# mosesyhc/LCGP

Hardware: AMD Instinct MI355X
Metric: NLL+grad evals/sec (higher is better)
Workload: dtype f64; 1 GPU; configs[2]: n=4096 d=6 p=64 q=8 submethod=full, one NLL+gradient evaluation per step; n=4096, d=6, p=64, q=8, parallelism=latent components k -> rank k mod 1, q_local_rank0=8

## Files before the change

### include/lcgp_hip.h

```cpp
#ifndef LCGP_HIP_H
#define LCGP_HIP_H

#include <stddef.h>
#include <stdint.h>

#ifdef __cplusplus
extern "C" {
#endif

#define LCGP_F64 0
#define LCGP_F32 1

#define LCGP_KERNEL_MATERN32 0
#define LCGP_KERNEL_SE 1
#define LCGP_KERNEL_MATERN52 2

int lcgp_version(void);
const char* lcgp_source_hash(void);
const char* lcgp_last_error(void);

int lcgp_theta_width(int d, int p);
int lcgp_out_width(int d, int p);
int lcgp_partial_width(int d, int p, int q_total);

typedef struct lcgp_sched {
    int outer_blocks;
    int syrk_small_tiles;
    int trtri_small_tiles;
    int lauum_small_tiles;
    int trtri_level_small;
    int fill_leaf;
    int fill_step;
    int leaf_in_wide;
    int progressive_tiles;
    int progressive_far;
    int progressive_lauum;
    int pair_tiles;
} lcgp_sched;
int lcgp_sched_default(lcgp_sched* sched );

int lcgp_workspace_bytes(int dtype, int n, int d, int p, int q_local, size_t* bytes );
int lcgp_predict_scratch_bytes(int dtype, int n, int q_local, int n0, size_t* bytes );

int lcgp_matern32(void* stream, int dtype, int n1, int n2, int d,
                  const void* x1, const void* x2,
                  const double* ell , double scale, double nug, int same, void* out);
int lcgp_covmat(void* stream, int dtype, int kernel_id, int n1, int n2, int d,
                const void* x1, const void* x2,
                const double* ell , double scale, double nug, int same, void* out);

int lcgp_kernel_build(void* stream, int dtype, int kernel_id, int n, int d, int p, int q_local,
                      const void* x , const void* sr ,
                      const double* theta, void* workspace);

int lcgp_potrf_logdet(void* stream, int dtype, int n, int d, int p, int q_local, void* workspace,
                      double* half_logdet, int* info, const lcgp_sched* sched ,
                      const void* plan );

int lcgp_potri(void* stream, int dtype, int n, int d, int p, int q_local, void* workspace,
               const lcgp_sched* sched);
// ... 288 lines not shown
```

### lcgp_amd/_hip.py

```python
from __future__ import annotations

import ctypes as C
import os
import subprocess

_HERE = os.path.dirname(os.path.abspath(__file__))
_ROOT = os.path.dirname(_HERE)
LIB_PATH = os.environ.get("LCGP_HIP_LIB") or os.path.join(_HERE, "liblcgp_hip.so")
SRC_PATH = os.path.join(_HERE, "csrc", "lcgp_hip.hip")
HDR_PATH = os.path.join(_ROOT, "include", "lcgp_hip.h")
SCHED_PATH = os.path.join(_HERE, "csrc", "fill_sched.h")
SUBSET_PATH = os.path.join(_HERE, "csrc", "sobol_subset.h")

F64, F32 = 0, 1
KERNELS = {"matern32": 0, "se": 1, "matern52": 2}


class Sched(C.Structure):
    _fields_ = [("outer_blocks", C.c_int), ("syrk_small_tiles", C.c_int), ("trtri_small_tiles", C.c_int),
                ("lauum_small_tiles", C.c_int), ("trtri_level_small", C.c_int), ("fill_leaf", C.c_int),
                ("fill_step", C.c_int), ("leaf_in_wide", C.c_int), ("progressive_tiles", C.c_int), ("progressive_far", C.c_int), ("progressive_lauum", C.c_int), ("pair_tiles", C.c_int)]


_vp, _i, _d = C.c_void_p, C.c_int, C.c_double
_sp = C.POINTER(Sched)
SIGNATURES = {
    "lcgp_version": (_i, []),
    "lcgp_source_hash": (C.c_char_p, []),
    "lcgp_last_error": (C.c_char_p, []),
    "lcgp_theta_width": (_i, [_i, _i]),
    "lcgp_out_width": (_i, [_i, _i]),
    "lcgp_partial_width": (_i, [_i, _i, _i]),
    "lcgp_sched_default": (_i, [_sp]),
    "lcgp_workspace_bytes": (_i, [_i, _i, _i, _i, _i, C.POINTER(C.c_size_t)]),
    "lcgp_predict_scratch_bytes": (_i, [_i, _i, _i, _i, C.POINTER(C.c_size_t)]),
    "lcgp_matern32": (_i, [_vp, _i, _i, _i, _i, _vp, _vp, C.POINTER(_d), _d, _d, _i, _vp]),
    "lcgp_covmat": (_i, [_vp, _i, _i, _i, _i, _i, _vp, _vp, C.POINTER(_d), _d, _d, _i, _vp]),
    "lcgp_kernel_build": (_i, [_vp, _i, _i, _i, _i, _i, _i, _vp, _vp, _vp, _vp]),
    "lcgp_potrf_logdet": (_i, [_vp, _i, _i, _i, _i, _i, _vp, _vp, _vp, _sp, _vp]),
    "lcgp_potri": (_i, [_vp, _i, _i, _i, _i, _i, _vp, _sp]),
    "lcgp_trtri": (_i, [_vp, _i, _i, _i, _i, _i, _vp, _sp]),
    "lcgp_lauum": (_i, [_vp, _i, _i, _i, _i, _i, _vp, _sp]),
    "lcgp_lauum_clock": (_i, [_vp, _i, _i, _i, _i, _i, _vp, _vp]),
    "lcgp_fetch_matrix": (_i, [_vp, _i, _i, _i, _i, _i, _vp, _i, _i, _vp]),
# ... 178 lines not shown
```

### lcgp_amd/csrc/fill_sched.h

```cpp
#ifndef LCGP_FILL_SCHED_H
#define LCGP_FILL_SCHED_H

#include <stddef.h>
#include <string.h>
#include <utility>
#include <vector>

namespace lcgp_fill {

enum FillType { FILL_NONE = 0, FILL_SYRK = 1, FILL_BROW = 2, FILL_CUPD = 3, FILL_DUPD = 4, FILL_TRI_T = 5, FILL_TRI_W = 6 };

constexpr int NJ = 6;

struct FillJob {
    int type;
    int nblk;
    int t0;
    int R0, R1, j0, j1;
    int kb0, kb1;
};

struct FillSet {
    void* M; void* W; void* V;
    size_t mat;
// ... 171 lines not shown
                fs.nblk += o.nblk;
            }
            hi = lo;
            jb.next = jb.total;
        }
        return fs.nblk;
    }

    void end_launch() {
        for (QJob& jb : jobs) jb.avail = jb.next;
        ++launch;
    }
};

struct PlanParams {
    int nb;
    int q;
    int ob;
    int syrk_small_tiles, fill_leaf, fill_step, leaf_in_wide;
    bool progressive;
    bool far_rides;
    bool with_dupd = true;
    int pair_tiles = 0;
};

enum LaunchKind {
    L_LEAF = 1,
    L_STEP = 2,
    L_TRAIL = 3,
    L_FILL = 4
};

struct Launch {
    Launch() { memset((void*)this, 0, sizeof(*this)); }
    int kind = 0;
    int J = 0, pe = 0, c = 0;
    int diag_end = 0, has_special = 0, n_trmm = 0, n_upd = 0;
    int c_lo = 0, c_hi = 0, tiles128 = 0, with_leaf = 0;
    FillSet fs;
};

inline long rect_tiles(int nb, int c_lo, int c_hi) { return syrk_tiles(nb / 2, c_lo, c_hi); }
inline int trapezoid_tiles(int nb, int c_lo, int c_hi) { return (c_hi - c_lo) * nb - (c_lo + c_hi - 1) * (c_hi - c_lo) / 2; }

class Planner {
 public:
    explicit Planner(const PlanParams& p) : pp(p) { fq.q = p.q; }
    std::vector<Launch> launches;
    bool inverse_planned = false;

    void run() {
        const int nb = pp.nb, ob = pp.ob, q = pp.q;
        const bool t128 = (ob & 1) == 0;
        inverse_planned = pp.progressive;
        bool leaf_done = false;
        const int cap_with_leaf = pp.fill_leaf + (ob - 1) * pp.fill_step;
        const int cap_no_leaf = (ob - 1) * pp.fill_step;
        for (int J = 0; J < nb; J += ob) {
            const int pe = J + ob < nb ? J + ob : nb;
            const int mid = pe + ob < nb ? pe + ob : nb;
            auto first_filler_column = [&](int cap_blocks) {
// ... 38 lines not shown
            panel(J, pe, leaf_done, next_leaf);
            if (pe >= nb) break;
            if (pe < c_hi) {
                Launch l;
                l.kind = L_TRAIL; l.J = k_lo; l.pe = pe; l.c_lo = pe; l.c_hi = c_hi;
                l.tiles128 = t128 && (long long)q * trapezoid_tiles(nb / 2, pe / 2, c_hi / 2) >= pp.syrk_small_tiles ? 1 : 0;
                l.with_leaf = next_leaf ? 1 : 0;
                l.fs.njobs = 0; l.fs.nblk = 0;
                launches.push_back(l);
                fq.end_launch();
            }
            leaf_done = next_leaf && pe < c_hi;
            queue_far_update(J, pe, cf);
        }
        int guard = 0;
        while (fq.pending()) {
            Launch l;
            l.kind = L_FILL;
            fq.take_final(l.fs, kb_end);
            if (l.fs.nblk <= 0 || ++guard > 4 * nb + 16) { failed = true; return; }
            launches.push_back(l);
            fq.end_launch();
        }
    }
    bool failed = false;

 private:
    int pair_J = -1, pair_cf = 0;
    PlanParams pp;
    FillQueue fq;
    int urgent_row = 0;
    int last_dupd = -1, last_cupd = -1;
    int kb_end = 0;

    void queue_far_update(int J, int pe, int cf) {
        fq.syrk_job = -1;
        if (cf >= pp.nb) return;
        QJob jb;
        jb.j.type = FILL_SYRK;
        jb.j.R0 = 0; jb.j.R1 = pp.nb / 2; jb.j.j0 = cf; jb.j.j1 = pp.nb; jb.j.kb0 = J; jb.j.kb1 = pe;
        jb.total = syrk_tiles(pp.nb / 2, cf, pp.nb);
        jb.ready_launch = fq.launch;
        fq.syrk_job = fq.add(jb);
    }

    void queue_inverse_jobs(int J, int pe, bool last_step) {
        const int nb = pp.nb;
        const int now = fq.launch;
        int prev = -1;
        for (int mb = 1; mb < pp.ob; mb *= 2) {
// ... 100 lines not shown
```

### lcgp_amd/csrc/lcgp_hip.hip

```cpp
#include <hip/hip_runtime.h>
#include <stdint.h>
#include <stdio.h>
#include <string.h>
#include <math.h>
#include <type_traits>
#include <vector>

#include "../../include/lcgp_hip.h"
#include "fill_sched.h"
#include "sobol_subset.h"

#define LCGP_VERSION 610

namespace {

constexpr int TS = 64;
constexpr int KT = 16;
constexpr int DMAX = 32;
constexpr int DWIDE = 126;

typedef double d4 __attribute__((ext_vector_type(4)));
typedef float f4 __attribute__((ext_vector_type(4)));

thread_local char g_err[256] = "";
// ... 471 lines not shown
    double o;
    asm("s_nop 1\n\tv_mov_b64_dpp %0, %1 row_newbcast:%2 row_mask:0xf bank_mask:0xf" : "=v"(o) : "v"(x), "n"(C));
    return o;
}

template <int C>
__device__ __forceinline__ void fmac_row_bcast(double& acc, double u, double v) {
    asm("v_fmac_f64_dpp %0, %1, %2 row_newbcast:%3 row_mask:0xf bank_mask:0xf" : "+v"(acc) : "v"(u), "v"(v), "n"(C));
}

template <int S, int C>
struct PivotCols {
    static __device__ __forceinline__ void run(double (&rD)[16], double (&rL)[16], double vD, double vL) {
        if constexpr (C < 16) {
            fmac_row_bcast<C>(rD[C], rD[S], vD);
            fmac_row_bcast<C>(rL[C], rD[S], vL);
            PivotCols<S, C + 1>::run(rD, rL, vD, vL);
        }
    }
};

template <int S>
struct PivotSteps {
    static __device__ __forceinline__ void run(double (&rD)[16], double (&rL)[16], double& dmine, int i) {
        if constexpr (S < 16) {
            const double dp = row_bcast<S>(rD[S]);
            dmine = i == S ? rD[S] : dmine;
            const double rdp = fast_rcp(dp);
            const double vD = -rD[S] * rdp, vL = -rL[S] * rdp;
            PivotCols<S, S + 1>::run(rD, rL, vD, vL);
            PivotSteps<S + 1>::run(rD, rL, dmine, i);
        }
    }
};

template <int S>
struct ScaleCols {
    static __device__ __forceinline__ void run(double (&rD)[16], double (&rL)[16], double rsl) {
        if constexpr (S < 16) {
            const double f = row_bcast<S>(rsl);
            rD[S] *= f;
            rL[S] *= f;
            ScaleCols<S + 1>::run(rD, rL, rsl);
        }
    }
};

__device__ __forceinline__ double fast_rsqrt(double a) {
    double y = __builtin_amdgcn_rsq(a);
    double e = fma(-(a * y), y, 1.0);
    y = fma(0.5 * y, e, y);
    e = fma(-(a * y), y, 1.0);
    y = fma(0.5 * y, e, y);
    return y;
// ... 75 lines not shown
            acc[rb][e] = rb < wv ? 0.0 : FROM_LDS ? w[rb * 16 + lq + 4 * e][wv * 16 + li]
                                                  : (double)Mb[(size_t)(rb * 16 + lq + 4 * e) * npad + wv * 16 + li];
    double (*S)[17] = (double (*)[17])scratch;
    int first_bad = 0;
#pragma unroll 1
    for (int kb = 0; kb < 4; ++kb) {
        if (wv == kb) {
#pragma unroll
            for (int rb = 0; rb < 4; ++rb)
#pragma unroll
                for (int e = 0; e < 4; ++e)
                    if (rb >= kb) S[rb * 16 + lq + 4 * e][li] = acc[rb][e];
            const int nlow = 3 - kb;
            const int base = kb * 16;
            double rD[16], rL[16];
            const int lrow = lq < nlow ? base + 16 * (1 + lq) + li : base + li;
#pragma unroll
            for (int c = 0; c < 16; ++c) {
                rD[c] = S[base + li][c];
                const double below = S[lrow][c];
                rL[c] = lq < nlow ? below : 0.0;
            }
            double dmine = 1.0;
            PivotSteps<0>::run(rD, rL, dmine, li);
            const double rsl = fast_rsqrt(dmine);
            ScaleCols<0>::run(rD, rL, rsl);
            if (lq == 0) { dinv[base + li] = rsl; pivs[base + li] = dmine; }
            const unsigned long long bm = __ballot(!(dmine > 0.0)) & 0xffffull;
            if (bm) first_bad = jb * TS + base + __ffsll((long long)bm);
            const int row = lq < nlow ? base + 16 * (1 + lq) + li : lq == nlow ? base + li : 16 * (lq - nlow - 1) + li;
#pragma unroll
            for (int m = 0; m < 16; ++m)
                lt[base + m][row] = lq < nlow ? rL[m] : (lq == nlow && li >= m) ? rD[m] : 0.0;
            if (lane == 0) bad[kb] = first_bad;
        } else if (wv == kb - 1) {
            const int a = kb - 1;
            leaf_inverse_diag(lt, w, dinv, a, lane);
            for (int b = 0; b < a; ++b) {
                const d4 tacc = leaf_inverse_t(lt, w, a, b, lane);
                leaf_inverse_w(w, tacc, a, b, lane);
            }
        } else if (kb == 0) {
            if ((jb & 1) == 0)
                for (int i = wv - 1; i < TS; i += 3) Wb[(size_t)i * npad + TS + lane] = (T)0;
        } else if (wv == ((kb + 1) & 3)) {
            leaf_store_l_panel<T>(Mb, npad, lt, kb - 1, lane);
        } else if (kb >= 2 && wv == ((kb + 2) & 3)) {
// ... 52 lines not shown

template <typename T>
__global__ __launch_bounds__(256, 2) void leaf_kernel(T* __restrict__ M, T* __restrict__ W, size_t mat, int npad, int jb,
                                                   double* __restrict__ logdet, int* __restrict__ info) {
    __shared__ __align__(16) unsigned char lds[LEAF_LDS_BYTES];
    leaf_body<T>(lds, blockIdx.x, M, W, mat, npad, jb, logdet, info);
}

enum GemmOp { OP_SYRK = 1, OP_TRTRI_T = 2, OP_TRTRI_W = 3, OP_LAUUM = 4, OP_PRED_U = 5, OP_PRED_COV = 6, OP_PRED_V = 7, OP_VR = 8,
              OP_VG_P = 9, OP_VG_G = 10, OP_HESS_G = 11, OP_COND_CROSS = 12, OP_COND_U = 13 };
enum Lay { MK = 0, KM = 1 };

struct GemmArgs {
    const void* A; const void* B; void* C;
    size_t sA, sB, sC;
    int ldA, ldB, ldC;
    int nb;
    int p0, p1, p2, p3;
    int q;
    int t0;
    int skipq;
    const void* bvec = nullptr;
    double* part = nullptr;
    unsigned long long* clk = nullptr;
    const double* theta = nullptr;
    const void* xa = nullptr;
    const void* xb = nullptr;
    const double* wref = nullptr;
    const double* gvc = nullptr;
    int ldg = 0, d = 0, kern = 0, tw = 0, nrep = 1, ldp = 0;
};

template <typename T>
__device__ __forceinline__ constexpr int lds_swz(int k) { return (k & 12) * (int)(8 / sizeof(T)); }
static_assert(KT == 16, "lds_swz assumes 16 k rows per stage");
template <typename T>
__device__ __forceinline__ int swz_col(int g16, int l15, int kk) {
    return (g16 ^ (lds_swz<T>(4 * kk) & ~15)) + (l15 ^ (lds_swz<T>(4 * kk) & 15));
}

template <typename T, int L, int TM, int NT>
__device__ __forceinline__ void load_stage(const T* __restrict__ P, int ld, int ks, T (&reg)[TM * KT / NT], int tid) {
    constexpr int EPT = TM * KT / NT;
    if (L == MK) {
        constexpr int TPR = KT / EPT;
        const int m = tid / TPR, kk = (tid % TPR) * EPT;
// ... 220 lines not shown
            }
        }
#pragma unroll
    for (int ni = 0; ni < MIN; ++ni) {
        s[ni] += __shfl_xor(s[ni], 16);
        s[ni] += __shfl_xor(s[ni], 32);
    }
    if (wave >= 2 && lane < 16) {
#pragma unroll
        for (int ni = 0; ni < MIN; ++ni) red[wn0 + ni * 16 + l15] = s[ni];
    }
    __syncthreads();
    if (wave < 2 && lane < 16) {
        const double rd = 1.0 / (D * (double)g.nrep);
        double* part = (double*)g.C + ((size_t)k * ((g.p2 + TM - 1) / TM) + rt) * g.ldp;
#pragma unroll
        for (int ni = 0; ni < MIN; ++ni) {
            const int cl = wn0 + ni * 16 + l15, c = c0 + cl;
            if (c < g.p3) part[c] = (s[ni] + red[cl]) / (fmax(g.gvc[(size_t)k * g.ldg + c], 0.0) + rd);
        }
    }
}

template <typename T, int OP, int TM, int NW>
__device__ __forceinline__ void gemm_body(const GemmArgs& g, const int lin ,
                                          unsigned char* lds) {
    constexpr int LA = (OP == OP_LAUUM) ? KM : MK;
    constexpr int LB = (OP == OP_TRTRI_T || OP == OP_TRTRI_W || OP == OP_LAUUM || OP == OP_PRED_V || OP == OP_VG_G || OP == OP_HESS_G ||
                        OP == OP_COND_U) ? KM : MK;
    constexpr int NT = NW * 64;
    constexpr int LD = TM + 16;
    constexpr int WTM = TM / (NW / 2), WTN = TM / 2;
    constexpr int MIM = WTM / 16, MIN = WTN / 16;
    constexpr int EPT = TM * KT / NT;
    T* As = (T*)lds;
    T* Bs = As + 2 * KT * LD;

    int lin_ = lin;
    if constexpr (OP == OP_TRTRI_T || OP == OP_TRTRI_W || OP == OP_LAUUM) {
        if (g.q < 4 && !g.skipq && ((lin >> 8) & 1)) {
            const int base = lin & ~255, nblk = (int)gridDim.x;
            const int top = base + 255 < nblk ? base + 255 : nblk - 1;
            lin_ = top - (lin - base);
        }
    }
    const int k = lin_ % g.q;
    const int bid = lin_ / g.q;
    const T* Ab = (const T*)g.A + (size_t)k * g.sA;
    const T* Bb = (const T*)g.B + (size_t)k * g.sB;
    T* Cb = (T*)g.C + (size_t)k * g.sC;

    const T* A0; const T* B0; T* Ct;
    ptrdiff_t dA, dB;
    int nkt;
    double alpha = 1.0;
    bool accumulate = false;
    bool tri_b = false;
    if constexpr (OP == OP_SYRK) {
        constexpr int SB = 8;
        int t = bid + g.t0, r;
        int i0 = 0;
        for (;;) {
            const int rows = g.nb - g.p2 - i0 < SB ? g.nb - g.p2 - i0 : SB;
            int cnt = 0;
            for (int i = i0; i < i0 + rows; ++i) cnt += (i < g.p3 - g.p2 ? i : g.p3 - g.p2 - 1) + 1;
            if (t < cnt) break;
            t -= cnt;
            i0 += SB;
        }
        const int rows = g.nb - g.p2 - i0 < SB ? g.nb - g.p2 - i0 : SB;
        int j = 0;
        for (;;) {
            const int lo = j > i0 ? j : i0;
            const int cnt = i0 + rows - lo;
            if (t < cnt) { r = g.p2 + lo + t; break; }
            t -= cnt;
            ++j;
        }
        const int c = g.p2 + j;
        A0 = Ab + (size_t)r * TM * g.ldA + (size_t)g.p0 * TM; dA = TM;
        B0 = Bb + (size_t)c * TM * g.ldB + (size_t)g.p0 * TM; dB = TM;
        nkt = g.p1 - g.p0;
        Ct = Cb + (size_t)r * TM * g.ldC + (size_t)c * TM;
        alpha = -1.0; accumulate = true;
    } else if constexpr (OP == OP_TRTRI_T || OP == OP_TRTRI_W) {
        const int mb = g.p0;
        const int npair = g.p1;
        const int pr = g.p2 + bid % npair, rem = bid / npair;
        int rl, cl;
        if constexpr (OP == OP_TRTRI_T) { cl = rem / mb; rl = rem - cl * mb; }
        else { rl = mb - 1 - rem / mb; cl = rem % mb; }
        const int C0 = 2 * pr * mb, R0 = C0 + mb;
        if (R0 + rl >= g.nb) return;
        if constexpr (OP == OP_TRTRI_T) {
            A0 = Ab + (size_t)(R0 + rl) * TM * g.ldA + (size_t)(C0 + mb - 1) * TM; dA = -(ptrdiff_t)TM;
            B0 = Bb + (size_t)(C0 + mb - 1) * TM * g.ldB + (size_t)(C0 + cl) * TM; dB = -(ptrdiff_t)TM * g.ldB;
            nkt = mb - cl;
        } else {
            A0 = Ab + (size_t)(R0 + rl) * TM * g.ldA + (size_t)R0 * TM; dA = TM;
            B0 = Bb + (size_t)R0 * TM * g.ldB + (size_t)(C0 + cl) * TM; dB = (ptrdiff_t)TM * g.ldB;
            nkt = rl + 1;
            alpha = -1.0;
        }
        Ct = Cb + (size_t)(R0 + rl) * TM * g.ldC + (size_t)(C0 + cl) * TM;
    } else if constexpr (OP == OP_LAUUM) {
        int r, c;
// ... 229 lines not shown
    }
    if constexpr (OP == OP_VR) {
        const int ct = bid % g.p1, rt = bid / g.p1;
        if (g.kern == 0) vr_epilogue<T, 0, TM, MIM, MIN>(g, acc, k, rt, ct, tid, wm0, wn0, lds);
        else if (g.kern == 1) vr_epilogue<T, 1, TM, MIM, MIN>(g, acc, k, rt, ct, tid, wm0, wn0, lds);
        else vr_epilogue<T, 2, TM, MIM, MIN>(g, acc, k, rt, ct, tid, wm0, wn0, lds);
        return;
    }
    if constexpr (OP == OP_PRED_COV) alpha = -g.theta[(size_t)k * g.p1 + g.p2];
    if constexpr (OP == OP_COND_CROSS) alpha = -g.theta[(size_t)k * g.p2 + g.p3];
#pragma unroll
    for (int mi = 0; mi < MIM; ++mi)
#pragma unroll
        for (int ni = 0; ni < MIN; ++ni)
#pragma unroll
            for (int e = 0; e < 4; ++e) {
                const unsigned dvoff = cvoff + ni * 16 * (unsigned)sizeof(T), dsoff = c_soff(mi, e);
                if constexpr (OP == OP_SYRK && TM == 128) {
                    if (g.skipq && bid + g.t0 == 0 && wm0 + mi * 16 + Mfma<T>::row(lane, e) < TS && wn0 + ni * 16 + (lane & 15) < TS)
                        continue;
                }
                if constexpr (PRELOAD_C) {
                    BufIo<T>::store((T)acc[mi][ni][e], crs, dvoff, dsoff);
                } else {
                    double v = alpha * (double)acc[mi][ni][e];
                    if (accumulate) v += (double)BufIo<T>::load(crs, dvoff, dsoff);
                    BufIo<T>::store((T)v, crs, dvoff, dsoff);
                }
            }
    if constexpr (OP == OP_LAUUM || OP == OP_SYRK) {
        if (g.clk && lin == 0 && wave == 0) {
            const unsigned long long c1 = __builtin_amdgcn_s_memtime() - clk0, r1 = __builtin_amdgcn_s_memrealtime() - rt0;
            if (lane == 0) { g.clk[0] = c1; g.clk[1] = r1; }
        }
    }
    if constexpr (OP == OP_LAUUM && TM == 128) {
        if (g.part) {
            __syncthreads();
            double* bsh = (double*)lds;
            double* p1s = bsh + 256;
            double* p2s = p1s + 256;
            int r, c;
            tri_decode(bid, r, c);
            const T* bk = (const T*)g.bvec + (size_t)k * g.ldC;
            if (tid < 256) bsh[tid] = (double)bk[(size_t)(tid < 128 ? r : c) * 128 + (tid & 127)];
            __syncthreads();
// ... 189 lines not shown
        const int ks = own ? 2 * R : kb0;
        rect_tile<T, KM, KM, false>(W + (size_t)ks * TS * ld + (size_t)R * 128, ld, W + (size_t)ks * TS * ld + (size_t)j * TS, ld,
                                    V + (size_t)R * 128 * ld + (size_t)j * TS, ld, (kb1 - ks) * (TS / KT), own, lds);
    }
}

constexpr int FILL_LDS_BYTES = 2 * KT * (128 + 16 + 64 + 16) * 8;

template <typename T>
__global__ __launch_bounds__(256, 2) void fill_kernel(FillSet fs) {
    __shared__ __align__(16) unsigned char lds[FILL_LDS_BYTES];
    fill_dispatch<T>(fs, blockIdx.x, lds);
}

template <typename T>
__global__ __launch_bounds__(256, 2) void leaf_fill_kernel(T* __restrict__ M, T* __restrict__ W, size_t mat, int npad, int jb,
                                                        double* __restrict__ logdet, int* __restrict__ info,
                                                        int q, FillSet fs) {
    __shared__ __align__(16) unsigned char lds[LEAF_LDS_BYTES];
    if ((int)blockIdx.x < q) leaf_body<T>(lds, blockIdx.x, M, W, mat, npad, jb, logdet, info);
    else fill_dispatch<T>(fs, blockIdx.x - q, lds);
}

struct StepArgs {
    void* M; void* W; size_t mat; int npad; int nb;
    int c, J, pe;
    int diag_end;
    int q;
    int has_special;
    int n_trmm;
    int n_upd;
    int trmm_r0, upd_r0;
    double* logdet; int* info;
    FillSet fs;
};

template <typename T>
struct Tile64 {
    typedef typename Mfma<T>::acc_t acc_t;
    static constexpr int LD = TS + 16, NT = 256, EPT = TS * KT / NT, SPT = TS / KT;
    static __device__ __forceinline__ void load(acc_t (&acc)[2][2], const T* Ct, int ld, int lane, int wm0, int wn0) {
#pragma unroll
        for (int i = 0; i < 2; ++i)
#pragma unroll
            for (int j = 0; j < 2; ++j)
#pragma unroll
                for (int e = 0; e < 4; ++e)
                    acc[i][j][e] = Ct[(size_t)(wm0 + i * 16 + Mfma<T>::row(lane, e)) * ld + wn0 + j * 16 + (lane & 15)];
    }
    static __device__ __forceinline__ void zero(acc_t (&acc)[2][2]) {
#pragma unroll
        for (int i = 0; i < 2; ++i)
#pragma unroll
            for (int j = 0; j < 2; ++j)
#pragma unroll
                for (int e = 0; e < 4; ++e) acc[i][j][e] = 0;
    }
    static __device__ __forceinline__ void store(const acc_t (&acc)[2][2], T* Ct, int ld, int lane, int wm0, int wn0) {
#pragma unroll
// ... 26 lines not shown
                T af[2], bf[2];
#pragma unroll
                for (int i = 0; i < 2; ++i) {
                    const T v = as[krow + wm0 + swz_col<T>(i * 16, lane & 15, kk)];
                    af[i] = NEG ? -v : v;
                }
#pragma unroll
                for (int j = 0; j < 2; ++j) bf[j] = bs[krow + wn0 + swz_col<T>(j * 16, lane & 15, kk)];
#pragma unroll
                for (int i = 0; i < 2; ++i)
#pragma unroll
                    for (int j = 0; j < 2; ++j) acc[i][j] = Mfma<T>::run(af[i], bf[j], acc[i][j]);
            }
        }
    }
    template <bool NEG>
    static __device__ __forceinline__ void mma(acc_t (&acc)[2][2], const T* A0, int ldA, const T* B0, int ldB, T* lds,
                                               int tid, int lane, int wm0, int wn0) {
        T pa[SPT][EPT], pb[SPT][EPT];
        fetch(pa, A0, ldA, tid);
        fetch(pb, B0, ldB, tid);
        mma_regs<NEG>(acc, pa, pb, lds, tid, lane, wm0, wn0);
    }
    static __device__ __forceinline__ void to_operand(const acc_t (&acc)[2][2], T* F, int lane, int wm0, int wn0) {
#pragma unroll
        for (int i = 0; i < 2; ++i)
#pragma unroll
            for (int j = 0; j < 2; ++j)
#pragma unroll
                for (int e = 0; e < 4; ++e)
                    F[(wn0 + j * 16 + (lane & 15)) * LD + ((wm0 + i * 16 + Mfma<T>::row(lane, e)) ^ (lane & 15))] = acc[i][j][e];
    }
    template <bool NEG>
    static __device__ __forceinline__ void mma_a_lds(acc_t (&acc)[2][2], const T* F, const T (&pb)[SPT][EPT], T* Bs, int tid,
                                                     int lane, int wm0, int wn0) {
#pragma unroll
        for (int s = 0; s < SPT; ++s) {
            store_stage<T, MK, TS, NT>(Bs + (s & 1) * KT * LD, pb[s], tid);
            __syncthreads();
            const T* as = F + s * KT * LD;
            const T* bs = Bs + (s & 1) * KT * LD;
#pragma unroll
            for (int kk = 0; kk < KT / 4; ++kk) {
                const int krow = (kk * 4 + (lane >> 4)) * LD;
                T af[2], bf[2];
#pragma unroll
                for (int i = 0; i < 2; ++i) {
                    const T v = as[krow + wm0 + i * 16 + ((lane & 15) ^ (4 * kk + (lane >> 4)))];
                    af[i] = NEG ? -v : v;
                }
#pragma unroll
                for (int j = 0; j < 2; ++j) bf[j] = bs[krow + wn0 + swz_col<T>(j * 16, lane & 15, kk)];
#pragma unroll
                for (int i = 0; i < 2; ++i)
#pragma unroll
                    for (int j = 0; j < 2; ++j) acc[i][j] = Mfma<T>::run(af[i], bf[j], acc[i][j]);
            }
        }
    }
    template <bool NEG>
    static __device__ __forceinline__ void mma_ab_lds(acc_t (&acc)[2][2], const T* F, int lane, int wm0, int wn0) {
#pragma unroll
        for (int kk = 0; kk < TS / 4; ++kk) {
            const int krow = (kk * 4 + (lane >> 4)) * LD;
            T af[2], bf[2];
#pragma unroll
            for (int i = 0; i < 2; ++i) {
                const T v = F[krow + wm0 + i * 16 + ((lane & 15) ^ ((4 * kk + (lane >> 4)) & 15))];
                af[i] = NEG ? -v : v;
            }
#pragma unroll
            for (int j = 0; j < 2; ++j) bf[j] = F[krow + wn0 + j * 16 + ((lane & 15) ^ ((4 * kk + (lane >> 4)) & 15))];
#pragma unroll
            for (int i = 0; i < 2; ++i)
#pragma unroll
                for (int j = 0; j < 2; ++j) acc[i][j] = Mfma<T>::run(af[i], bf[j], acc[i][j]);
        }
    }
};

template <typename T>
__device__ __forceinline__ void chain_step_body(const StepArgs& a, int b, unsigned char* lds) {
    typedef Tile64<T> TL;
    const int tid = body_tid(), lane = tid & 63, wave = __builtin_amdgcn_readfirstlane(tid >> 6);
    const int wm0 = (wave >> 1) * 32, wn0 = (wave & 1) * 32;
    const int ld = a.npad;
    const int nspecial = a.has_special * a.q;
    int t = -1, k = 0;
    if (b < nspecial) { t = 0; k = b; }
    else if (b < nspecial + a.fs.nblk) { fill_dispatch<T>(a.fs, b - nspecial, lds); return; }
    else {
        b -= nspecial + a.fs.nblk;
        if (b < (a.n_trmm - a.has_special) * a.q) { k = b % a.q; t = b / a.q + a.has_special; }
        else b -= (a.n_trmm - a.has_special) * a.q;
    }
    if (t >= 0) {
        if (t == 0 && a.has_special) __builtin_amdgcn_s_setprio(3);
        const int c = a.c, r = a.trmm_r0 + t;
        T* Mk = (T*)a.M + (size_t)k * a.mat;
        const T* Wk = (const T*)a.W + (size_t)k * a.mat;
        T* Ct = Mk + (size_t)r * TS * ld + (size_t)c * TS;
        T* F = (T*)lds;
// ... 55 lines not shown
            if (j + 1 < a.c) {
                TL::fetch(pa[1], Ar + (size_t)(j + 1) * TS, ld, tid);
                TL::fetch(pb[1], Br + (size_t)(j + 1) * TS, ld, tid);
            }
            TL::template mma_regs<true>(acc, pa[0], pb[0], (T*)lds, tid, lane, wm0, wn0);
            if (j + 1 < a.c) {
                if (j + 2 < a.c) {
                    TL::fetch(pa[0], Ar + (size_t)(j + 2) * TS, ld, tid);
                    TL::fetch(pb[0], Br + (size_t)(j + 2) * TS, ld, tid);
                }
                TL::template mma_regs<true>(acc, pa[1], pb[1], (T*)lds, tid, lane, wm0, wn0);
            }
        }
        TL::store(acc, Ct, ld, lane, wm0, wn0);
    }
}

template <typename T>
__global__ __launch_bounds__(256, 2) void chain_step_kernel(StepArgs a) {
    __shared__ __align__(16) unsigned char lds[LEAF_LDS_BYTES];
    chain_step_body<T>(a, blockIdx.x, lds);
}

template <typename T, int TM>
__global__ __launch_bounds__(256, 2) void wide_leaf_kernel(GemmArgs g, T* __restrict__ M, T* __restrict__ W, size_t mat,
                                                           int npad, int jb, double* __restrict__ logdet,
                                                           int* __restrict__ info) {
    constexpr int WIDE_LDS = 4 * KT * (TM + 16) * (int)sizeof(T);
    __shared__ __align__(16) unsigned char lds[WIDE_LDS > LEAF_LDS_BYTES ? WIDE_LDS : LEAF_LDS_BYTES];
    const int q = g.q;
    if ((int)blockIdx.x < q) {
        leaf_body<T>(lds, blockIdx.x, M, W, mat, npad, jb, logdet, info);
        return;
    }
    gemm_body<T, OP_SYRK, TM, 4>(g, blockIdx.x - q, lds);
}

template <typename T>
__global__ __launch_bounds__(256) void symv_tile_kernel(const T* __restrict__ V, size_t mat, int npad,
                                                        const T* __restrict__ b, double* __restrict__ part, int ntile) {
    __shared__ double vt[TS][TS + 1];
    __shared__ double red[4][TS];
    __shared__ double br[TS], bc[TS];
    const int k = blockIdx.y;
    int r, c;
    tri_decode(blockIdx.x, r, c);
    const T* Vt = V + (size_t)k * mat + (size_t)r * TS * npad + (size_t)c * TS;
    const int tid = threadIdx.x, j = tid & 63, g = tid >> 6;
    if (tid < TS) {
        br[tid] = (double)b[(size_t)k * npad + r * TS + tid];
        bc[tid] = (double)b[(size_t)k * npad + c * TS + tid];
    }
    double v[16];
#pragma unroll
    for (int m = 0; m < 16; ++m) v[m] = (double)Vt[(size_t)(g * 16 + m) * npad + j];
    __syncthreads();
    double* dst = part + ((size_t)k * ntile + blockIdx.x) * 2 * TS;
    double s2 = 0.0;
// ... 818 lines not shown
    GemmArgs h = g;
    h.q = q;
    h.t0 = 0;
    h.skipq = 0;
    hipLaunchKernelGGL((tile_gemm<T, OP, TM, NW>), dim3((unsigned)ntiles * q), dim3(NW * 64), 0, st, h);
    CHECK_LAUNCH("tile_gemm");
    return 0;
}

inline lcgp_sched default_sched() {
    lcgp_sched s;
    s.outer_blocks = 0;
    s.syrk_small_tiles = 3000;
    s.trtri_small_tiles = 4200;
    s.lauum_small_tiles = 2048;
    s.trtri_level_small = 600;
    s.fill_leaf = 248;
    s.fill_step = 248;
    s.leaf_in_wide = 2048;
    s.progressive_tiles = 600;
    s.progressive_far = 1;
    s.progressive_lauum = 48;
    s.pair_tiles = 4000;
    return s;
}

inline int check_sched(const lcgp_sched& s) {
    if (s.outer_blocks < 0 || s.outer_blocks > 64) return bad("sched.outer_blocks must be in [0, 64]");
    if (s.syrk_small_tiles < 0 || s.trtri_small_tiles < 0 || s.lauum_small_tiles < 0 || s.trtri_level_small < 0 ||
        s.fill_leaf < 0 || s.fill_step < 0 || s.leaf_in_wide < 0 || s.progressive_tiles < 0 || s.progressive_lauum < 0 ||
        s.pair_tiles < 0)
        return bad("sched fields must be >= 0");
    return 0;
}

using lcgp_fill::trapezoid_tiles;

template <typename T>
int launch_fill(hipStream_t st, const FillSet& fs) {
    if (fs.nblk <= 0) return 0;
    hipLaunchKernelGGL((fill_kernel<T>), dim3((unsigned)fs.nblk), dim3(256), 0, st, fs);
    CHECK_LAUNCH("fill_kernel");
    return 0;
}

template <typename T>
int potrf_trailing(hipStream_t st, const Ws& w, int J, int pe, int c_lo, int c_hi, bool tiles128, bool with_leaf,
                   unsigned long long* clk = nullptr) {
    if (c_lo >= c_hi) return 0;
    T* M = (T*)(w.base + w.off_M);
    GemmArgs g;
    g.sA = g.sB = g.sC = w.mat; g.ldA = g.ldB = g.ldC = w.npad;
    g.A = M; g.B = M; g.C = M;
    g.clk = clk;
    if (tiles128) {
        g.nb = w.nb / 2; g.p0 = J / 2; g.p1 = pe / 2; g.p2 = c_lo / 2; g.p3 = c_hi / 2;
        const int nt = trapezoid_tiles(w.nb / 2, c_lo / 2, c_hi / 2);
        if (with_leaf) {
            g.q = w.q; g.t0 = 0; g.skipq = 1;
            hipLaunchKernelGGL((wide_leaf_kernel<T, 128>), dim3((unsigned)(nt + 1) * w.q), dim3(256), 0, st, g, M,
                               (T*)(w.base + w.off_W), w.mat, w.npad, c_lo, (double*)(w.base + w.off_logdet),
                               (int*)(w.base + w.off_info));
            CHECK_LAUNCH("wide_leaf_kernel");
            return 0;
        }
        return launch_gemm<T, OP_SYRK, 128>(st, g, nt, w.q);
    }
    g.nb = w.nb; g.p0 = J; g.p1 = pe; g.p2 = c_lo; g.p3 = c_hi;
    const int nt = trapezoid_tiles(w.nb, c_lo, c_hi);
    if (with_leaf) {
        g.q = w.q; g.t0 = 1; g.skipq = 0;
        hipLaunchKernelGGL((wide_leaf_kernel<T, 64>), dim3((unsigned)nt * w.q), dim3(256), 0, st, g, M,
                           (T*)(w.base + w.off_W), w.mat, w.npad, c_lo, (double*)(w.base + w.off_logdet),
                           (int*)(w.base + w.off_info));
        CHECK_LAUNCH("wide_leaf_kernel");
        return 0;
    }
    return launch_gemm<T, OP_SYRK>(st, g, nt, w.q);
}

constexpr unsigned PLAN_MAGIC = 0x4c43504cu;
struct PlanHeader {
    unsigned magic;
    int version;
    int dtype, n, nb, q, with_inverse;
    int nlaunch;
    int inverse_done;
    int reserved;
    lcgp_sched sched;
    size_t off_launch, bytes;
};

inline lcgp_fill::PlanParams plan_params(int dtype, int nb, int q, bool with_inverse, const lcgp_sched& sc, int* inverse_done) {
    lcgp_fill::PlanParams pp;
    pp.nb = nb; pp.q = q;
    pp.ob = sc.outer_blocks < 1 ? (dtype == LCGP_F32 ? 8 : 4) : sc.outer_blocks;
    pp.syrk_small_tiles = sc.syrk_small_tiles; pp.fill_leaf = sc.fill_leaf; pp.fill_step = sc.fill_step;
    pp.leaf_in_wide = sc.leaf_in_wide;
    bool prog = false;
    if (with_inverse && sc.progressive_tiles > 0 && pp.ob >= 2 && (pp.ob & (pp.ob - 1)) == 0) {
        const int nb2 = nb / 2;
        prog = (long long)q * (nb2 * (nb2 + 1) / 2) <= sc.progressive_tiles;
    }
    pp.progressive = prog;
    pp.far_rides = !(pp.progressive && sc.progressive_far == 0);
    pp.with_dupd = nb <= sc.progressive_lauum;
    pp.pair_tiles = sc.pair_tiles;
    if (inverse_done) *inverse_done = pp.progressive ? (pp.with_dupd ? 2 : 1) : 0;
    return pp;
}

inline size_t make_plan(int dtype, int n, int q, bool with_inverse, const lcgp_sched& sc, void* out,
                        std::vector<char>* vec = nullptr) {
    const int npad = round_up(n, 2 * TS), nb = npad / TS;
    int inverse_done = 0;
    lcgp_fill::Planner plan(plan_params(dtype, nb, q, with_inverse, sc, &inverse_done));
    plan.run();
    if (plan.failed) { bad("internal: the filler queue did not drain"); return 0; }
    PlanHeader h;
    memset(&h, 0, sizeof(h));
    h.magic = PLAN_MAGIC; h.version = LCGP_VERSION;
    h.dtype = dtype; h.n = n; h.nb = nb; h.q = q; h.with_inverse = with_inverse ? 1 : 0;
    h.nlaunch = (int)plan.launches.size();
    h.inverse_done = inverse_done;
    h.sched = sc;
    h.off_launch = (sizeof(PlanHeader) + 255) & ~size_t(255);
    h.bytes = (h.off_launch + sizeof(lcgp_fill::Launch) * h.nlaunch + 255) & ~size_t(255);
    if (vec) { vec->resize(h.bytes); out = vec->data(); }
    if (out) {
        memset(out, 0, h.bytes);
// ... 21 lines not shown
    if (!stats_zeroed) {
        hipLaunchKernelGGL(zero_stats_kernel, dim3((w.q + 63) / 64), dim3(64), 0, st, logdet, info, w.q);
        CHECK_LAUNCH("zero_stats");
    }
    const int dtype = sizeof(T) == 4 ? LCGP_F32 : LCGP_F64;
    std::vector<char> local;
    if (!plan_host) {
        if (!make_plan(dtype, w.n, w.q, with_inverse, sc, nullptr, &local)) return -1;
        plan_host = local.data();
    }
    const PlanHeader* h = (const PlanHeader*)plan_host;
    if (inverse_done) *inverse_done = h->inverse_done;
    const lcgp_fill::Launch* launches = (const lcgp_fill::Launch*)((const char*)plan_host + h->off_launch);
    const int nlaunch = h->nlaunch;
    bool first_trail = true;
    for (int li = 0; li < nlaunch; ++li) {
        const lcgp_fill::Launch& l = launches[li];
        FillSet fs = l.fs;
        fs.M = w.base + w.off_M; fs.W = w.base + w.off_W; fs.V = w.base + w.off_V;
        fs.mat = w.mat; fs.npad = w.npad; fs.nb = w.nb; fs.q = w.q;
        int rc = 0;
        switch (l.kind) {
            case lcgp_fill::L_LEAF:
                if (fs.nblk > 0)
                    hipLaunchKernelGGL((leaf_fill_kernel<T>), dim3(w.q + fs.nblk), dim3(256), 0, st, M, W, w.mat, w.npad, l.J,
                                       logdet, info, w.q, fs);
                else
                    hipLaunchKernelGGL((leaf_kernel<T>), dim3(w.q), dim3(256), 0, st, M, W, w.mat, w.npad, l.J, logdet, info);
                CHECK_LAUNCH("leaf_kernel");
                break;
            case lcgp_fill::L_STEP: {
                StepArgs a;
                a.M = M; a.W = W; a.mat = w.mat; a.npad = w.npad; a.nb = w.nb;
                a.c = l.c; a.J = l.J; a.pe = l.pe; a.q = w.q;
                a.diag_end = l.diag_end; a.has_special = l.has_special; a.n_trmm = l.n_trmm; a.n_upd = l.n_upd;
                a.trmm_r0 = l.c + 1;
                a.upd_r0 = l.c + 2;
                a.logdet = logdet; a.info = info;
                a.fs = fs;
                const long nblk = (long)(a.n_trmm + a.n_upd) * w.q + fs.nblk;
                hipLaunchKernelGGL((chain_step_kernel<T>), dim3((unsigned)nblk), dim3(256), 0, st, a);
                CHECK_LAUNCH("chain_step_kernel");
                break;
            }
            case lcgp_fill::L_TRAIL:
                rc = potrf_trailing<T>(st, w, l.J, l.pe, l.c_lo, l.c_hi, l.tiles128 != 0, l.with_leaf != 0,
                                       first_trail ? (unsigned long long*)(w.base + w.off_clock) : nullptr);
                first_trail = false;
                break;
            default:
                rc = launch_fill<T>(st, fs);
        }
        if (rc) return rc;
    }
    return 0;
}

inline bool use_small_tiles(const Ws& w, int threshold) {
    const int nb2 = w.nb / 2;
    return (long long)w.q * (nb2 * (nb2 + 1) / 2) < threshold;
}

template <typename T, int TM>
int trtri_level(hipStream_t st, const Ws& w, int mb) {
    GemmArgs g;
    g.sA = g.sB = g.sC = w.mat; g.ldA = g.ldB = g.ldC = w.npad; g.p2 = g.p3 = 0;
    const int nbt = w.npad / TM;
    g.nb = nbt;
    const int pairs = (nbt + 2 * mb - 1) / (2 * mb);
    g.p0 = mb; g.p1 = pairs;
// ... 5450 lines not shown
```

Before: 96.61 evals/s.

## Pre-apply next chain-step panel update inside current TRMM tile to shorten Cholesky chain

Adds a planner pass that marks consecutive small chain-step launches inside a diagonal block, letting one step's TRMM tile also apply the next column's update, using a saved copy of the pre-step tile in V. This moves one update tile off the serial critical path, so the following step can skip that work. It adds leaf_copy/duplicated-store paths and a new chain_pre_kernel with extra LDS use and extra GEMMs. Separately, the pivot loop in the leaf factorization now computes the next reciprocal early so the broadcast and reciprocal latency overlap with the remaining column updates.

```diff
diff --git a/include/lcgp_hip.h b/include/lcgp_hip.h
--- a/include/lcgp_hip.h
+++ b/include/lcgp_hip.h
@@ -36,6 +36,7 @@
     int progressive_far;
     int progressive_lauum;
     int pair_tiles;
+    int pre_apply_tiles;
 } lcgp_sched;
 int lcgp_sched_default(lcgp_sched* sched );
 
diff --git a/lcgp_amd/_hip.py b/lcgp_amd/_hip.py
--- a/lcgp_amd/_hip.py
+++ b/lcgp_amd/_hip.py
@@ -19,7 +19,8 @@
 class Sched(C.Structure):
     _fields_ = [("outer_blocks", C.c_int), ("syrk_small_tiles", C.c_int), ("trtri_small_tiles", C.c_int),
                 ("lauum_small_tiles", C.c_int), ("trtri_level_small", C.c_int), ("fill_leaf", C.c_int),
-                ("fill_step", C.c_int), ("leaf_in_wide", C.c_int), ("progressive_tiles", C.c_int), ("progressive_far", C.c_int), ("progressive_lauum", C.c_int), ("pair_tiles", C.c_int)]
+                ("fill_step", C.c_int), ("leaf_in_wide", C.c_int), ("progressive_tiles", C.c_int), ("progressive_far", C.c_int), ("progressive_lauum", C.c_int), ("pair_tiles", C.c_int),
+                ("pre_apply_tiles", C.c_int)]
 
 
 _vp, _i, _d = C.c_void_p, C.c_int, C.c_double
diff --git a/lcgp_amd/csrc/fill_sched.h b/lcgp_amd/csrc/fill_sched.h
--- a/lcgp_amd/csrc/fill_sched.h
+++ b/lcgp_amd/csrc/fill_sched.h
@@ -217,6 +217,7 @@
     bool far_rides;
     bool with_dupd = true;
     int pair_tiles = 0;
+    int pre_apply_tiles = 0;
 };
 
 enum LaunchKind {
@@ -232,6 +233,9 @@
     int J = 0, pe = 0, c = 0;
     int diag_end = 0, has_special = 0, n_trmm = 0, n_upd = 0;
     int c_lo = 0, c_hi = 0, tiles128 = 0, with_leaf = 0;
+    int pre_do = 0;
+    int pre_done = 0;
+    int pre_copy = 0;
     FillSet fs;
 };
 
@@ -316,10 +320,39 @@
             launches.push_back(l);
             fq.end_launch();
         }
+        mark_pre_applied();
     }
     bool failed = false;
 
  private:
+    void mark_pre_applied() {
+        if (pp.pre_apply_tiles <= 0) return;
+        const int n = (int)launches.size();
+        std::vector<char> quiet(n, 0);
+        for (int i = 0; i < n; ++i) {
+            const Launch& l = launches[i];
+            quiet[i] = l.kind == L_STEP && l.fs.nblk == 0 && (long long)(l.n_trmm + l.n_upd) * pp.q <= pp.pre_apply_tiles;
+        }
+        for (int i = 1; i < n; ++i) {
+            if (launches[i].kind != L_STEP || launches[i].c != launches[i].J) continue;
+            Launch& before = launches[i - 1];
+            const int J = launches[i].J;
+            const bool can_copy = (before.kind == L_LEAF && before.J == J && before.fs.nblk == 0) ||
+                                  (before.kind == L_TRAIL && before.with_leaf && !before.tiles128 && before.c_lo == J);
+            if (!can_copy) continue;
+            for (int j = i; j + 1 < n; ++j) {
+                Launch& s = launches[j];
+                Launch& nx = launches[j + 1];
+                if (nx.kind != L_STEP || nx.J != J || nx.c != s.c + 1 || s.c + 2 >= s.pe) break;
+                if (!quiet[j] || !quiet[j + 1]) break;
+                s.pre_do = 1;
+                nx.pre_done = 1;
+                if (s.n_upd > 0) --s.n_upd;
+                if (j == i) before.pre_copy = 1;
+            }
+        }
+    }
+
     int pair_J = -1, pair_cf = 0;
     PlanParams pp;
     FillQueue fq;
diff --git a/lcgp_amd/csrc/lcgp_hip.hip b/lcgp_amd/csrc/lcgp_hip.hip
--- a/lcgp_amd/csrc/lcgp_hip.hip
+++ b/lcgp_amd/csrc/lcgp_hip.hip
@@ -517,14 +517,17 @@
 
 template <int S>
 struct PivotSteps {
-    static __device__ __forceinline__ void run(double (&rD)[16], double (&rL)[16], double& dmine, int i) {
+    static __device__ __forceinline__ void run(double (&rD)[16], double (&rL)[16], double& dmine, int i, double rdp) {
         if constexpr (S < 16) {
-            const double dp = row_bcast<S>(rD[S]);
             dmine = i == S ? rD[S] : dmine;
-            const double rdp = fast_rcp(dp);
             const double vD = -rD[S] * rdp, vL = -rL[S] * rdp;
-            PivotCols<S, S + 1>::run(rD, rL, vD, vL);
-            PivotSteps<S + 1>::run(rD, rL, dmine, i);
+            if constexpr (S + 1 < 16) {
+                fmac_row_bcast<S + 1>(rD[S + 1], rD[S], vD);
+                fmac_row_bcast<S + 1>(rL[S + 1], rD[S], vL);
+                const double rdn = fast_rcp(row_bcast<S + 1>(rD[S + 1]));
+                PivotCols<S, S + 2>::run(rD, rL, vD, vL);
+                PivotSteps<S + 1>::run(rD, rL, dmine, i, rdn);
+            }
         }
     }
 };
@@ -646,7 +649,7 @@
                 rL[c] = lq < nlow ? below : 0.0;
             }
             double dmine = 1.0;
-            PivotSteps<0>::run(rD, rL, dmine, li);
+            PivotSteps<0>::run(rD, rL, dmine, li, fast_rcp(row_bcast<0>(rD[0])));
             const double rsl = fast_rsqrt(dmine);
             ScaleCols<0>::run(rD, rL, rsl);
             if (lq == 0) { dinv[base + li] = rsl; pivs[base + li] = dmine; }
@@ -745,6 +748,7 @@
     int skipq;
     const void* bvec = nullptr;
     double* part = nullptr;
+    void* D = nullptr; size_t sD = 0;
     unsigned long long* clk = nullptr;
     const double* theta = nullptr;
     const void* xa = nullptr;
@@ -1011,7 +1015,7 @@
     }
 }
 
-template <typename T, int OP, int TM, int NW>
+template <typename T, int OP, int TM, int NW, bool DUP = false >
 __device__ __forceinline__ void gemm_body(const GemmArgs& g, const int lin ,
                                           unsigned char* lds) {
     constexpr int LA = (OP == OP_LAUUM) ? KM : MK;
@@ -1045,6 +1049,7 @@
     double alpha = 1.0;
     bool accumulate = false;
     bool tri_b = false;
+    [[maybe_unused]] T* Dt = nullptr;
     if constexpr (OP == OP_SYRK) {
         constexpr int SB = 8;
         int t = bid + g.t0, r;
@@ -1071,6 +1076,9 @@
         B0 = Bb + (size_t)c * TM * g.ldB + (size_t)g.p0 * TM; dB = TM;
         nkt = g.p1 - g.p0;
         Ct = Cb + (size_t)r * TM * g.ldC + (size_t)c * TM;
+        if constexpr (DUP) {
+            if (g.D && r == g.p2 + 1 && c == g.p2) Dt = (T*)g.D + (size_t)k * g.sD + (size_t)r * TM * g.ldC + (size_t)c * TM;
+        }
         alpha = -1.0; accumulate = true;
     } else if constexpr (OP == OP_TRTRI_T || OP == OP_TRTRI_W) {
         const int mb = g.p0;
@@ -1346,6 +1354,9 @@
                 }
                 if constexpr (PRELOAD_C) {
                     BufIo<T>::store((T)acc[mi][ni][e], crs, dvoff, dsoff);
+                    if constexpr (DUP) {
+                        if (Dt) BufIo<T>::store((T)acc[mi][ni][e], tile_rsrc(Dt), dvoff, dsoff);
+                    }
                 } else {
                     double v = alpha * (double)acc[mi][ni][e];
                     if (accumulate) v += (double)BufIo<T>::load(crs, dvoff, dsoff);
@@ -1581,6 +1592,21 @@
     else fill_dispatch<T>(fs, blockIdx.x - q, lds);
 }
 
+template <typename T>
+__global__ __launch_bounds__(256, 2) void leaf_copy_kernel(T* __restrict__ M, T* __restrict__ W, size_t mat, int npad, int jb,
+                                                        double* __restrict__ logdet, int* __restrict__ info, int q,
+                                                        T* __restrict__ V) {
+    __shared__ __align__(16) unsigned char lds[LEAF_LDS_BYTES];
+    if ((int)blockIdx.x < q) { leaf_body<T>(lds, blockIdx.x, M, W, mat, npad, jb, logdet, info); return; }
+    const int k = blockIdx.x - q, tid = body_tid();
+    const size_t off = (size_t)k * mat + (size_t)(jb + 1) * TS * npad + (size_t)jb * TS;
+#pragma unroll
+    for (int i = 0; i < TS * TS / 256; ++i) {
+        const size_t e = off + (size_t)((tid >> 6) + 4 * i) * npad + (tid & 63);
+        V[e] = M[e];
+    }
+}
+
 struct StepArgs {
     void* M; void* W; size_t mat; int npad; int nb;
     int c, J, pe;
@@ -1594,6 +1620,20 @@
     FillSet fs;
 };
 
+struct PreStepArgs {
+    StepArgs s;
+    void* V;
+    int pre_do;
+    int pre_done;
+};
+
+constexpr int PRE_LDG = TS + 8;
+template <typename T>
+constexpr int chain_lds_bytes() {
+    constexpr int two = (TS * (TS + 16) + TS * PRE_LDG) * (int)sizeof(T);
+    return two > LEAF_LDS_BYTES ? two : LEAF_LDS_BYTES;
+}
+
 template <typename T>
 struct Tile64 {
     typedef typename Mfma<T>::acc_t acc_t;
@@ -1666,6 +1706,7 @@
         fetch(pb, B0, ldB, tid);
         mma_regs<NEG>(acc, pa, pb, lds, tid, lane, wm0, wn0);
     }
+    template <int LDF = LD>
     static __device__ __forceinline__ void to_operand(const acc_t (&acc)[2][2], T* F, int lane, int wm0, int wn0) {
 #pragma unroll
         for (int i = 0; i < 2; ++i)
@@ -1673,7 +1714,7 @@
             for (int j = 0; j < 2; ++j)
 #pragma unroll
                 for (int e = 0; e < 4; ++e)
-                    F[(wn0 + j * 16 + (lane & 15)) * LD + ((wm0 + i * 16 + Mfma<T>::row(lane, e)) ^ (lane & 15))] = acc[i][j][e];
+                    F[(wn0 + j * 16 + (lane & 15)) * LDF + ((wm0 + i * 16 + Mfma<T>::row(lane, e)) ^ (lane & 15))] = acc[i][j][e];
     }
     template <bool NEG>
     static __device__ __forceinline__ void mma_a_lds(acc_t (&acc)[2][2], const T* F, const T (&pb)[SPT][EPT], T* Bs, int tid,
@@ -1702,6 +1743,25 @@
             }
         }
     }
+    template <bool NEG, int LDG>
+    static __device__ __forceinline__ void mma_fg_lds(acc_t (&acc)[2][2], const T* F, const T* G, int lane, int wm0, int wn0) {
+#pragma unroll
+        for (int kk = 0; kk < TS / 4; ++kk) {
+            const int kx = kk * 4 + (lane >> 4), sw = (lane & 15) ^ (kx & 15);
+            T af[2], bf[2];
+#pragma unroll
+            for (int i = 0; i < 2; ++i) {
+                const T v = F[kx * LD + wm0 + i * 16 + sw];
+                af[i] = NEG ? -v : v;
+            }
+#pragma unroll
+            for (int j = 0; j < 2; ++j) bf[j] = G[kx * LDG + wn0 + j * 16 + sw];
+#pragma unroll
+            for (int i = 0; i < 2; ++i)
+#pragma unroll
+                for (int j = 0; j < 2; ++j) acc[i][j] = Mfma<T>::run(af[i], bf[j], acc[i][j]);
+        }
+    }
     template <bool NEG>
     static __device__ __forceinline__ void mma_ab_lds(acc_t (&acc)[2][2], const T* F, int lane, int wm0, int wn0) {
 #pragma unroll
@@ -1722,6 +1782,87 @@
         }
     }
 };
+
+template <typename T, bool PRE>
+__device__ __forceinline__ void chain_trmm_tile(const PreStepArgs& pa, int t, int k, unsigned char* lds) {
+    typedef Tile64<T> TL;
+    const StepArgs& a = pa.s;
+    const int tid = body_tid(), lane = tid & 63, wave = __builtin_amdgcn_readfirstlane(tid >> 6);
+    const int wm0 = (wave >> 1) * 32, wn0 = (wave & 1) * 32;
+    const int ld = a.npad;
+    {
+        if (t == 0 && a.has_special) __builtin_amdgcn_s_setprio(3);
+        const int c = a.c, r = a.trmm_r0 + t;
+        T* Mk = (T*)a.M + (size_t)k * a.mat;
+        const T* Wk = (const T*)a.W + (size_t)k * a.mat;
+        T* Ct = Mk + (size_t)r * TS * ld + (size_t)c * TS;
+        T* F = (T*)lds;
+        T* Bst = F + TS * TL::LD;
+        typename TL::acc_t acc[2][2];
+        T pw[TL::SPT][TL::EPT];
+        TL::fetch(pw, Wk + (size_t)c * TS * ld + (size_t)c * TS, ld, tid);
+        [[maybe_unused]] typename TL::acc_t pacc[2][2];
+        if constexpr (PRE) {
+            TL::load(pacc, Ct + TS, ld, lane, wm0, wn0);
+            for (int j = a.J; j < c; ++j) {
+                TL::template mma<true>(pacc, Mk + (size_t)r * TS * ld + (size_t)j * TS, ld,
+                                       Mk + (size_t)(c + 1) * TS * ld + (size_t)j * TS, ld, (T*)lds, tid, lane, wm0, wn0);
+                __syncthreads();
+            }
+        }
+        TL::load(acc, Ct, ld, lane, wm0, wn0);
+        if (c > a.J && !(pa.pre_done && t == 0)) {
+            TL::template mma<true>(acc, Mk + (size_t)r * TS * ld + (size_t)(c - 1) * TS, ld,
+                                   Mk + (size_t)c * TS * ld + (size_t)(c - 1) * TS, ld, (T*)lds, tid, lane, wm0, wn0);
+            __syncthreads();
+        }
+        TL::to_operand(acc, F, lane, wm0, wn0);
+        TL::zero(acc);
+        TL::template mma_a_lds<false>(acc, F, pw, Bst, tid, lane, wm0, wn0);
+        TL::store(acc, Ct, ld, lane, wm0, wn0);
+        if (r < a.diag_end) {
+            T* Dt = Mk + (size_t)r * TS * ld + (size_t)r * TS;
+            typename TL::acc_t dacc[2][2];
+            TL::load(dacc, Dt, ld, lane, wm0, wn0);
+            __syncthreads();
+            TL::to_operand(acc, F, lane, wm0, wn0);
+            __syncthreads();
+            TL::template mma_ab_lds<true>(dacc, F, lane, wm0, wn0);
+            if (!PRE && a.has_special && t == 0) {
+                __syncthreads();
+                double (*blk)[LEAF_LDT] = (double (*)[LEAF_LDT])((double*)lds + TS * LEAF_LDT);
+#pragma unroll
+                for (int i = 0; i < 2; ++i)
+#pragma unroll
+                    for (int j = 0; j < 2; ++j)
+#pragma unroll
+                        for (int e = 0; e < 4; ++e)
+                            blk[wm0 + i * 16 + Mfma<T>::row(lane, e)][wn0 + j * 16 + (lane & 15)] = (double)dacc[i][j][e];
+                __syncthreads();
+                leaf_body<T, true>(lds, k, (T*)a.M, (T*)a.W, a.mat, a.npad, c + 1, a.logdet, a.info);
+            } else {
+                TL::store(dacc, Dt, ld, lane, wm0, wn0);
+            }
+        }
+        if constexpr (PRE) {
+            T* Vk = (T*)pa.V + (size_t)k * a.mat;
+            typename TL::acc_t xacc[2][2];
+            TL::load(xacc, Vk + (size_t)(c + 1) * TS * ld + (size_t)c * TS, ld, lane, wm0, wn0);
+            __syncthreads();
+            TL::to_operand(xacc, F, lane, wm0, wn0);
+            TL::zero(xacc);
+            TL::template mma_a_lds<false>(xacc, F, pw, Bst, tid, lane, wm0, wn0);
+            __syncthreads();
+            T* G = F + TS * TL::LD;
+            TL::to_operand(acc, F, lane, wm0, wn0);
+            TL::template to_operand<PRE_LDG>(xacc, G, lane, wm0, wn0);
+            __syncthreads();
+            TL::template mma_fg_lds<true, PRE_LDG>(pacc, F, G, lane, wm0, wn0);
+            TL::store(pacc, Ct + TS, ld, lane, wm0, wn0);
+            TL::store(pacc, Vk + (size_t)r * TS * ld + (size_t)(c + 1) * TS, ld, lane, wm0, wn0);
+        }
+    }
+}
 
 template <typename T>
 __device__ __forceinline__ void chain_step_body(const StepArgs& a, int b, unsigned char* lds) {
@@ -1823,6 +1964,37 @@
     chain_step_body<T>(a, blockIdx.x, lds);
 }
 
+template <typename T>
+__global__ __launch_bounds__(256, 2) void chain_pre_kernel(PreStepArgs pa) {
+    typedef Tile64<T> TL;
+    __shared__ __align__(16) unsigned char lds[chain_lds_bytes<T>()];
+    const StepArgs& a = pa.s;
+    const int tid = body_tid(), lane = tid & 63, wave = __builtin_amdgcn_readfirstlane(tid >> 6);
+    const int wm0 = (wave >> 1) * 32, wn0 = (wave & 1) * 32;
+    const int ld = a.npad;
+    int b = blockIdx.x;
+    if (b < a.n_trmm * a.q) {
+        const int first = a.has_special + pa.pre_do;
+        int t, k;
+        if (b < first * a.q) { t = b / a.q; k = b - t * a.q; }
+        else { b -= first * a.q; k = b % a.q; t = b / a.q + first; }
+        if (pa.pre_do && t == 1) chain_trmm_tile<T, true>(pa, t, k, lds);
+        else chain_trmm_tile<T, false>(pa, t, k, lds);
+        return;
+    }
+    b -= a.n_trmm * a.q;
+    const int k = b % a.q, t = b / a.q;
+    const int cc = a.c + 1, r = a.upd_r0 + t;
+    T* Mk = (T*)a.M + (size_t)k * a.mat;
+    T* Ct = Mk + (size_t)r * TS * ld + (size_t)cc * TS;
+    typename TL::acc_t acc[2][2];
+    TL::load(acc, Ct, ld, lane, wm0, wn0);
+    for (int j = a.J; j < a.c; ++j)
+        TL::template mma<true>(acc, Mk + (size_t)r * TS * ld + (size_t)j * TS, ld, Mk + (size_t)cc * TS * ld + (size_t)j * TS, ld,
+                               (T*)lds, tid, lane, wm0, wn0);
+    TL::store(acc, Ct, ld, lane, wm0, wn0);
+}
+
 template <typename T, int TM>
 __global__ __launch_bounds__(256, 2) void wide_leaf_kernel(GemmArgs g, T* __restrict__ M, T* __restrict__ W, size_t mat,
                                                            int npad, int jb, double* __restrict__ logdet,
@@ -1834,7 +2006,7 @@
         leaf_body<T>(lds, blockIdx.x, M, W, mat, npad, jb, logdet, info);
         return;
     }
-    gemm_body<T, OP_SYRK, TM, 4>(g, blockIdx.x - q, lds);
+    gemm_body<T, OP_SYRK, TM, 4, TM == 64>(g, blockIdx.x - q, lds);
 }
 
 template <typename T>
@@ -2699,6 +2871,7 @@
     s.progressive_far = 1;
     s.progressive_lauum = 48;
     s.pair_tiles = 4000;
+    s.pre_apply_tiles = 1 << 30;
     return s;
 }
 
@@ -2706,7 +2879,7 @@
     if (s.outer_blocks < 0 || s.outer_blocks > 64) return bad("sched.outer_blocks must be in [0, 64]");
     if (s.syrk_small_tiles < 0 || s.trtri_small_tiles < 0 || s.lauum_small_tiles < 0 || s.trtri_level_small < 0 ||
         s.fill_leaf < 0 || s.fill_step < 0 || s.leaf_in_wide < 0 || s.progressive_tiles < 0 || s.progressive_lauum < 0 ||
-        s.pair_tiles < 0)
+        s.pair_tiles < 0 || s.pre_apply_tiles < 0)
         return bad("sched fields must be >= 0");
     return 0;
 }
@@ -2723,8 +2896,9 @@
 
 template <typename T>
 int potrf_trailing(hipStream_t st, const Ws& w, int J, int pe, int c_lo, int c_hi, bool tiles128, bool with_leaf,
-                   unsigned long long* clk = nullptr) {
+                   unsigned long long* clk = nullptr, bool pre_copy = false) {
     if (c_lo >= c_hi) return 0;
+    if (pre_copy && (tiles128 || !with_leaf)) return bad("internal: plan asks for a tile copy from a launch that cannot make it");
     T* M = (T*)(w.base + w.off_M);
     GemmArgs g;
     g.sA = g.sB = g.sC = w.mat; g.ldA = g.ldB = g.ldC = w.npad;
@@ -2747,6 +2921,7 @@
     const int nt = trapezoid_tiles(w.nb, c_lo, c_hi);
     if (with_leaf) {
         g.q = w.q; g.t0 = 1; g.skipq = 0;
+        if (pre_copy) { g.D = w.base + w.off_V; g.sD = w.mat; }
         hipLaunchKernelGGL((wide_leaf_kernel<T, 64>), dim3((unsigned)nt * w.q), dim3(256), 0, st, g, M,
                            (T*)(w.base + w.off_W), w.mat, w.npad, c_lo, (double*)(w.base + w.off_logdet),
                            (int*)(w.base + w.off_info));
@@ -2783,6 +2958,7 @@
     pp.far_rides = !(pp.progressive && sc.progressive_far == 0);
     pp.with_dupd = nb <= sc.progressive_lauum;
     pp.pair_tiles = sc.pair_tiles;
+    pp.pre_apply_tiles = sc.pre_apply_tiles;
     if (inverse_done) *inverse_done = pp.progressive ? (pp.with_dupd ? 2 : 1) : 0;
     return pp;
 }
@@ -2850,7 +3026,11 @@
         int rc = 0;
         switch (l.kind) {
             case lcgp_fill::L_LEAF:
-                if (fs.nblk > 0)
+                if (l.pre_copy) {
+                    if (fs.nblk > 0) return bad("internal: plan asks for a tile copy from a diagonal-block launch with filler");
+                    hipLaunchKernelGGL((leaf_copy_kernel<T>), dim3(2 * w.q), dim3(256), 0, st, M, W, w.mat, w.npad, l.J, logdet, info,
+                                       w.q, (T*)(w.base + w.off_V));
+                } else if (fs.nblk > 0)
                     hipLaunchKernelGGL((leaf_fill_kernel<T>), dim3(w.q + fs.nblk), dim3(256), 0, st, M, W, w.mat, w.npad, l.J,
                                        logdet, info, w.q, fs);
                 else
@@ -2863,17 +3043,23 @@
                 a.c = l.c; a.J = l.J; a.pe = l.pe; a.q = w.q;
                 a.diag_end = l.diag_end; a.has_special = l.has_special; a.n_trmm = l.n_trmm; a.n_upd = l.n_upd;
                 a.trmm_r0 = l.c + 1;
-                a.upd_r0 = l.c + 2;
+                a.upd_r0 = l.c + 2 + l.pre_do;
                 a.logdet = logdet; a.info = info;
                 a.fs = fs;
                 const long nblk = (long)(a.n_trmm + a.n_upd) * w.q + fs.nblk;
-                hipLaunchKernelGGL((chain_step_kernel<T>), dim3((unsigned)nblk), dim3(256), 0, st, a);
+                if (l.pre_do || l.pre_done) {
+                    if (fs.nblk > 0) return bad("internal: plan marks a chain step with filler as pre-applied");
+                    PreStepArgs pa;
+                    pa.s = a; pa.V = w.base + w.off_V; pa.pre_do = l.pre_do; pa.pre_done = l.pre_done;
+                    hipLaunchKernelGGL((chain_pre_kernel<T>), dim3((unsigned)nblk), dim3(256), 0, st, pa);
+                } else
+                    hipLaunchKernelGGL((chain_step_kernel<T>), dim3((unsigned)nblk), dim3(256), 0, st, a);
                 CHECK_LAUNCH("chain_step_kernel");
                 break;
             }
             case lcgp_fill::L_TRAIL:
                 rc = potrf_trailing<T>(st, w, l.J, l.pe, l.c_lo, l.c_hi, l.tiles128 != 0, l.with_leaf != 0,
-                                       first_trail ? (unsigned long long*)(w.base + w.off_clock) : nullptr);
+                                       first_trail ? (unsigned long long*)(w.base + w.off_clock) : nullptr, l.pre_copy != 0);
                 first_trail = false;
                 break;
             default:
```

Measured after the change: 96.05 evals/s. No clear change (-0.6%).
